# JiaruiFeng/KP-GNN

Measured on AMD Instinct MI355X. Metric: graphs/sec KP-GIN fwd+bwd, ZINC-12k K=8 L=8 h=104, higher is better.
Workload: dtype f32; 1 GPU; ZINC-12k-shaped synthetic molecules, KPGINPlus K=8 L=8 h=104 kernel=spd geometric combine, fwd+bwd+Adam, L1 loss; global_batch=2048, nodes_per_batch=47450, khop_edges_per_batch=1018372, active_pairs_per_batch=1018372, parallelism=dp1, launch=hipGraph replay of fwd+bwd, batches=4 pre-staged batches cycled

## Files before the change

### include/kpgnn.h

```cpp
#ifndef KPGNN_H_
#define KPGNN_H_

#include <stddef.h>
#include <stdint.h>

#ifdef __cplusplus
extern "C" {
#endif

#define KPGNN_ABI_VERSION 1

#define KPGNN_OK 0
#define KPGNN_EINVAL (-1)
#define KPGNN_EHIP (-2)
#define KPGNN_ELIMIT (-3)

typedef void* kpgnn_stream_t;

int kpgnn_abi_version(void);
const char* kpgnn_last_error(void);

int kpgnn_device_info(int* cu_count, int* lds_bytes_per_block, int* wavefront, char* arch, int arch_len);


// ... 124 lines not shown
} kpgnn_agg_fwd_desc;

int kpgnn_aggregate_fwd(const kpgnn_agg_fwd_desc* d, kpgnn_stream_t stream);

typedef struct kpgnn_pull_gather_desc {
    int32_t N, K, D;
    int32_t K_csr;
    const int32_t* n_dyn;
    const int32_t* rowptr;
    const int32_t* col;
    const float* slab[16];
    int64_t slab_sn;
    const float* hinit;
    const float* hinit2;
    float* hout;
} kpgnn_pull_gather_desc;

int kpgnn_khop_pull_gather(const kpgnn_pull_gather_desc* d, kpgnn_stream_t stream);

int64_t kpgnn_agg_lds_launch_count(void);

typedef struct kpgnn_agg_bwd_desc {
    int32_t N, K, D, K_csr, mode, n_code0, n_codek, use_tables;
    const int32_t* rowptr_src;
    const int32_t* col_src;
    const uint16_t* code_src;
    const float* dis;
    const float* g;
    int64_t g_sn, g_sk;
    const float* eps;
// ... 460 lines not shown
```

### kp_gnn_amd/_lib.py

```python
import ctypes
import os

import torch

_PKG = os.path.dirname(os.path.abspath(__file__))
HIP_LIB_PATH = os.path.join(_PKG, "libkpgnn_hip.so")

MODE_GIN, MODE_GINPLUS, MODE_GCN, MODE_SUM = 0, 1, 2, 3

c_i32, c_i64, c_f32p, c_vp = ctypes.c_int32, ctypes.c_int64, ctypes.c_void_p, ctypes.c_void_p


MATH_AUTO, MATH_F32 = 0, 1
ELIMIT = -3
DENSE_MATH = MATH_AUTO


class KpgnnError(RuntimeError):
    pass


class AggFwdDesc(ctypes.Structure):
    _fields_ = [
        ("N", c_i32), ("K", c_i32), ("D", c_i32), ("K_csr", c_i32), ("mode", c_i32),
# ... 6 lines not shown
        ("out", c_vp), ("o_sn", c_i64), ("o_sk", c_i64),
        ("pre", c_vp), ("theta", c_vp), ("hout", c_vp), ("xbias", c_vp),
        ("ptab", c_vp), ("uid", c_vp), ("uid_stride", c_i64),
        ("x_slot", c_vp * 16), ("n_dict", c_i32), ("alphas", c_vp), ("storage", c_i32),
        ("n_dyn", c_vp),
        ("graph_ptr", c_vp), ("num_graphs", c_i32), ("max_graph_nodes", c_i32), ("hinit", c_vp), ("hinit2", c_vp),
    ]


class PullGatherDesc(ctypes.Structure):
    _fields_ = [
        ("N", c_i32), ("K", c_i32), ("D", c_i32), ("K_csr", c_i32),
        ("n_dyn", c_vp), ("rowptr", c_vp), ("col", c_vp),
        ("slab", c_vp * 16), ("slab_sn", c_i64),
        ("hinit", c_vp), ("hinit2", c_vp), ("hout", c_vp),
    ]


class AggBwdDesc(ctypes.Structure):
    _fields_ = [
        ("N", c_i32), ("K", c_i32), ("D", c_i32), ("K_csr", c_i32), ("mode", c_i32),
        ("n_code0", c_i32), ("n_codek", c_i32), ("use_tables", c_i32),
        ("rowptr_src", c_vp), ("col_src", c_vp), ("code_src", c_vp), ("dis", c_vp),
        ("g", c_vp), ("g_sn", c_i64), ("g_sk", c_i64),
        ("eps", c_vp),
        ("gx", c_vp), ("gx_sn", c_i64), ("gx_sk", c_i64),
        ("gtable0", c_vp), ("gtablek", c_vp),
        ("gx_slot", c_vp * 16), ("accumulate_mask", ctypes.c_uint32), ("storage", c_i32),
        ("n_dyn", c_vp),
    ]
# ... 451 lines not shown
```

### kp_gnn_amd/csrc/aggregate.hip

```cpp
#include <initializer_list>

#include "kpgnn_common.h"

namespace kpgnn {
namespace {

constexpr int kBlock = 256;
constexpr int kMaxLdsTableBytes = 96 * 1024;

template <int VEC> struct V {
    float v[VEC];
    __device__ __forceinline__ static V zero() { V r; for (int i = 0; i < VEC; ++i) r.v[i] = 0.f; return r; }
    __device__ __forceinline__ static V load(const float* p) { V r; ldv<VEC>(p, r.v); return r; }
    __device__ __forceinline__ void store(float* p) const { stv<VEC>(p, v); }
    __device__ __forceinline__ void store_stream(float* p) const {
        for (int i = 0; i < VEC; ++i) __builtin_nontemporal_store(v[i], p + i);
    }
    template <bool BF> __device__ __forceinline__ static V load_row(const char* p) {
        if (BF) { V r; ld_bf16<VEC>(p, r.v); return r; }
        return load(reinterpret_cast<const float*>(p));
    }
    __device__ __forceinline__ void add(const V& o) { for (int i = 0; i < VEC; ++i) v[i] += o.v[i]; }
    __device__ __forceinline__ void fma(float s, const V& o) { for (int i = 0; i < VEC; ++i) v[i] = fmaf(s, o.v[i], v[i]); }
};
// ... 16 lines not shown
    const float* periph; int64_t p_sn, p_sk;
    const float* eps;
    float* out; int64_t o_sn, o_sk;
    float* pre;
    const float* theta;
    const float* alphas;
    float* theta_out;
    float* hout;
    const float* hinit;
    const float* hinit2;
    const float* xbias;
    const float* ptab; const int32_t* uid; int64_t uid_stride;
    const float* xs[16];
    int lds_theta, lds_ptab;
};

#ifndef KPGNN_PULL_WAVES
#define KPGNN_PULL_WAVES 7
#endif
#ifndef KPGNN_PULL_PF
#define KPGNN_PULL_PF 4
#endif
template <int VEC, int G, bool GCN, int TAB, bool FAST = false, bool BF = false, bool PULL = false>
__global__ void __launch_bounds__(kBlock, PULL ? KPGNN_PULL_WAVES : FAST ? 5 : 4)
agg_fwd_kernel(const FwdParams p) {
    static_assert(!PULL || (!GCN && TAB == 0 && !FAST && !BF), "the pull form gathers fp32 slabs without tables");
    const int N_live = live_rows(p.N, p.n_dyn);
    const int MODE = PULL ? (int)KPGNN_MODE_SUM : FAST ? (int)KPGNN_MODE_GINPLUS : p.mode;
    const bool COMBINE = (FAST || PULL) ? true : p.combine != 0;
    extern __shared__ __attribute__((aligned(16))) float lds_tab[];
    const int D = p.D;
    const float* thp = p.theta;
    const float* ptp = p.ptab;
    if (TAB == 1) {
        const int n0 = p.n_code0 * D, nk = p.n_codek * D;
        for (int t = threadIdx.x; t < n0; t += kBlock) lds_tab[t] = p.table0[t];
        for (int t = threadIdx.x; t < nk; t += kBlock) lds_tab[n0 + t] = p.tablek[t];
        float* th_l = lds_tab + ((n0 + nk + 3) & ~3);
        float* pt_l = th_l + ((p.lds_theta + 3) & ~3);
        if (p.alphas) {
            for (int d = threadIdx.x; d < D; d += kBlock) {
// ... 11 lines not shown
                    th_l[k * D + d] = th;
                    if (blockIdx.x == 0) p.theta_out[(int64_t)k * D + d] = th;
                    pw *= q;
                }
            }
        } else
        for (int t = threadIdx.x; t < p.lds_theta; t += kBlock) th_l[t] = p.theta[t];
        for (int t = threadIdx.x; t < p.lds_ptab; t += kBlock) pt_l[t] = p.ptab[t];
        if (p.lds_theta) thp = th_l;
        if (p.lds_ptab) ptp = pt_l;
        __syncthreads();
    }
    const float* tab0 = TAB == 1 ? lds_tab : p.table0;
    const float* tabk = TAB == 1 ? lds_tab + p.n_code0 * D : p.tablek;

    constexpr int NODES = kBlock / G;
    const int sg = threadIdx.x / G;
    const int sl = threadIdx.x % G;
    const int lane = threadIdx.x & (kWave - 1);
    const int sg_lane0 = lane - sl;
    const int c0 = sl * VEC;
    const bool col_ok = c0 < D;
    const float eps1 = 1.0f + (!PULL && p.eps ? p.eps[0] : 0.0f);
    const int64_t num_tiles = ((int64_t)N_live + NODES - 1) / NODES;
    constexpr uint32_t XB = BF ? 2u : 4u;
    const uint32_t xrow_b = (uint32_t)p.x_sn * XB, trow_b = (uint32_t)D * 4u;
    const uint32_t lane_b = col_ok ? (uint32_t)c0 * 4u : 0u;
    const uint32_t lane_bx = col_ok ? (uint32_t)c0 * XB : 0u;

    int last_u = -1;
    V<VEC> prow = V<VEC>::zero();
    for (XcdTileWalk w(num_tiles); w.valid(); w.next()) {
        const int64_t i = w.cur * NODES + sg;
        if (i >= N_live) continue;
        const int32_t* rp = p.rowptr + i * p.K_csr;
        V<VEC> hsum = V<VEC>::zero();
        if (!FAST && p.hinit && col_ok) hsum = V<VEC>::load(p.hinit + i * (int64_t)D + c0);
        if (!FAST && p.hinit2 && col_ok) hsum.add(V<VEC>::load(p.hinit2 + i * (int64_t)D + c0));
        const bool lane_meta = PULL ? true : G > p.K;
        int myrp = 0, myuid = 0;
        if (lane_meta) {
            myrp = rp[sl <= p.K ? sl : p.K];
            if (!PULL && (FAST || (p.uid && !p.periph))) myuid = p.uid[i * p.uid_stride + (sl < p.K ? sl : 0)];
        }
        int beg = lane_meta ? __shfl(myrp, sg_lane0) : rp[0];
        const int end_all = lane_meta ? __shfl(myrp, sg_lane0 + p.K) : rp[p.K];
        int cbase = beg;
        uint32_t coff = 0, ctab = 0;
        if (!GCN) {
            const int idx = cbase + sl;
            if (idx < end_all) {
                coff = (uint32_t)p.col[idx] * xrow_b;
                if (TAB != 0) ctab = (uint32_t)p.code[idx] * trow_b;
// ... 149 lines not shown
                if (FAST) v.add(V<VEC>::load(ptp + (int64_t)u * D + c0));
                else { if (u != last_u) { prow = V<VEC>::load(ptp + (int64_t)u * D + c0); last_u = u; } v.add(prow); }
            }
            if (MODE == KPGNN_MODE_GIN) { V<VEC> xs = V<VEC>::load(xk + i * p.x_sn); xs.add(xb); v.fma(eps1, xs); }
            if (COMBINE) {
                if (!FAST && !thp) hsum.add(v);
                else {
                    const V<VEC> th = V<VEC>::load(thp + k * D + c0);
                    for (int q = 0; q < VEC; ++q) hsum.v[q] = fmaf(th.v[q], v.v[q], hsum.v[q]);
                }
            } else {
                v.store_stream(p.out + i * p.o_sn + (int64_t)k * p.o_sk + c0);
            }
        }
        if (COMBINE && col_ok) hsum.store_stream(p.hout + i * (int64_t)D + c0);
    }
}

struct BwdParams {
    const int32_t* n_dyn;
    int N, K, D, K_csr, n_code0, n_codek, mode, bf;
    const int32_t* rowptr;
    const int32_t* col;
    const uint16_t* code;
    const float* dis;
    const float* g; int64_t g_sn, g_sk;
    const float* eps;
    float* gx; int64_t gx_sn, gx_sk;
    float* gtable0;
    float* gtablek;
// ... 183 lines not shown
    }
    if (TAB == 1) {
        __syncthreads();
        for (int t = threadIdx.x; t < n0; t += kBlock) { const float v = lds_gt[t]; if (v != 0.f) atomicAdd(p.gtable0 + t, v); }
        for (int t = threadIdx.x; t < nk; t += kBlock) { const float v = lds_gt[n0 + t]; if (v != 0.f) atomicAdd(p.gtablek + t, v); }
    }
}

unsigned pick_grid(int64_t num_tiles, int blocks_per_cu) {
    const int64_t cap = (int64_t)device_facts().cu_count * blocks_per_cu;
    int64_t g = num_tiles < cap ? num_tiles : cap;
    if (g >= kNumXcd) g = g / kNumXcd * kNumXcd;
    return (unsigned)(g > 0 ? g : 1);
}

template <int VEC, int G, bool GCN, int TAB, bool FAST = false, bool BF = false, bool PULL = false>
int launch_fwd(const FwdParams& p, size_t lds, hipStream_t s) {
    const int64_t tiles = ((int64_t)p.N + (kBlock / G) - 1) / (kBlock / G);
    if (lds > 64 * 1024)
        KPGNN_HIP_TRY(ensure_dynamic_lds((const void*)agg_fwd_kernel<VEC, G, GCN, TAB, FAST, BF, PULL>, lds));
    int nb = resident_blocks(agg_fwd_kernel<VEC, G, GCN, TAB, FAST, BF, PULL>, kBlock, lds);
    if (PULL && nb > KPGNN_PULL_WAVES) nb = KPGNN_PULL_WAVES;
    const unsigned grid = pick_grid(tiles, nb > 0 ? nb : 4);
    hipLaunchKernelGGL((agg_fwd_kernel<VEC, G, GCN, TAB, FAST, BF, PULL>), dim3(grid), dim3(kBlock), lds, s, p);
    KPGNN_LAUNCH_CHECK("agg_fwd_kernel");
    return KPGNN_OK;
}

template <int VEC, int G>
int launch_fwd_mode(const FwdParams& p, int tab, size_t lds, hipStream_t s) {
    const bool gcn = p.mode == KPGNN_MODE_GCN;
    const bool fast = tab == 1 && p.mode == KPGNN_MODE_GINPLUS && p.combine && !p.periph && p.uid && p.ptab && p.pre;
    if (p.bf) {
        if constexpr (VEC == 4) {
            if (fast && !p.x) return launch_fwd<VEC, G, false, 1, true, true>(p, lds, s);
        }
        return fail(KPGNN_EINVAL, "aggregate_fwd: bf16 storage needs the fused KP-GIN+ epilogue (GELU, theta, dictionary P, "
                    "code tables in LDS, S saved), per-hop inputs and D %% 4 == 0");
    }
// ... 132 lines not shown
    return dispatch_row_shape<64>(vec, row_lanes(d->D, vec), "aggregate_fwd",
                                  [&](auto VV, auto G) { return launch_fwd_mode<VV.value, G.value>(p, tab, lds, s); });
}

extern "C" int kpgnn_khop_pull_gather(const kpgnn_pull_gather_desc* d, kpgnn_stream_t stream) {
    KPGNN_REQUIRE(d != nullptr, "khop_pull_gather: NULL descriptor");
    KPGNN_REQUIRE(d->N >= 0 && d->K >= 1 && d->K <= 16 && d->D >= 1 && d->K_csr >= d->K, "khop_pull_gather: bad N=%d K=%d D=%d K_csr=%d",
                  d->N, d->K, d->D, d->K_csr);
    if ((int64_t)d->N * d->K_csr >= ((int64_t)1 << 31)) return fail(KPGNN_ELIMIT, "khop_pull_gather: N*K exceeds int32");
    if (d->N == 0) return KPGNN_OK;
    KPGNN_REQUIRE(d->rowptr != nullptr, "khop_pull_gather: NULL rowptr");
    KPGNN_REQUIRE(d->hout != nullptr, "khop_pull_gather: NULL output");
    for (int k = 0; k < d->K; ++k) KPGNN_REQUIRE(d->slab[k] != nullptr, "khop_pull_gather: NULL slab[%d]", k);
    if ((uint64_t)d->N * (uint64_t)d->slab_sn * 4u >= (1ull << 32))
        return fail(KPGNN_ELIMIT, "khop_pull_gather: N * slab row stride = %lld floats exceeds the 32-bit byte offsets of the gather", (long long)d->N * d->slab_sn);
    FwdParams p = {};
    p.N = d->N; p.n_dyn = d->n_dyn; p.K = d->K; p.D = d->D; p.K_csr = d->K_csr;
    p.mode = KPGNN_MODE_SUM; p.combine = 1;
    p.rowptr = d->rowptr; p.col = d->col;
    p.x_sn = d->slab_sn;
    p.hout = d->hout; p.hinit = d->hinit; p.hinit2 = d->hinit2;
    uintptr_t slot_bits = 0;
    for (int k = 0; k < d->K; ++k) {
        p.xs[k] = d->slab[k];
        slot_bits |= (uintptr_t)p.xs[k] & 15;
    }
    const void* slot_align = (const void*)(slot_bits | 16);
    const int vec = row_vec(d->D, {slot_align, d->hout, d->hinit, d->hinit2}, {d->slab_sn});
    const int lanes = (d->D + vec - 1) / vec;
    if (lanes > 64) return fail(KPGNN_ELIMIT, "khop_pull_gather: D=%d with %d-wide access needs %d lanes > 64", d->D, vec, lanes);
    hipStream_t s = (hipStream_t)stream;
    return dispatch_row_shape<64>(vec, row_lanes(d->D, vec), "khop_pull_gather", [&](auto VV, auto G) {
        if constexpr (VV.value == 4 && G.value >= 16) {
            if (G.value > d->K) return launch_fwd<4, G.value, false, 0, false, false, true>(p, 0, s);
        }
        return launch_fwd<VV.value, G.value, false, 0>(p, 0, s);
    });
}

extern "C" int kpgnn_aggregate_bwd(const kpgnn_agg_bwd_desc* d, kpgnn_stream_t stream) {
    KPGNN_REQUIRE(d != nullptr, "aggregate_bwd: NULL descriptor");
    KPGNN_REQUIRE(d->N >= 0 && d->K >= 1 && d->D >= 1 && d->K_csr >= d->K, "aggregate_bwd: bad N=%d K=%d D=%d K_csr=%d",
                  d->N, d->K, d->D, d->K_csr);
    if ((int64_t)d->N * d->K_csr >= ((int64_t)1 << 31)) return fail(KPGNN_ELIMIT, "aggregate_bwd: N*K exceeds int32");
    if (d->N == 0) return KPGNN_OK;
    KPGNN_REQUIRE(d->rowptr_src && d->g, "aggregate_bwd: NULL rowptr/g");
    if (!d->gx) {
// ... 51 lines not shown
```

### kp_gnn_amd/ops.py

```python
import ctypes

import torch

from . import _lib
from ._lib import MODE_GCN, MODE_GIN, MODE_GINPLUS, MODE_SUM, LaunchTimer, set_launch_timer

_SQRT1_2 = 0.7071067811865476
_INV_SQRT_2PI = 0.3989422804014327


def algorithmic_bytes(csr, k_act, D, n_tensors, n_rows_tables, extra_nd=0, s=4):
    A = csr.active_pairs(k_act)
    return int(s * csr.N * k_act * D * n_tensors) + A * 6 + 4 * (csr.N * csr.K + 1) + 4 * D * n_rows_tables \
        + 4 * csr.N * D * extra_nd


_STORAGE = torch.float32


def set_storage_dtype(dtype):
    global _STORAGE
    prev = _STORAGE
    dtype = {"fp32": torch.float32, "f32": torch.float32, "bf16": torch.bfloat16}.get(dtype, dtype)
    if dtype not in (torch.float32, torch.bfloat16):
# ... 195 lines not shown
        n_t = 1 + (periph is not None) + (pre is not None) + (theta is None)
        extra = 4 * N * K if uid is not None else 0
        return extra + algorithmic_bytes(csr, K, D, n_t, d.n_code0 + d.n_codek, extra_nd=1 if theta is not None else 0,
                                         s=2 if bf16 else 4)
    _lib.launch("kpgnn_aggregate_fwd", dev, ctypes.byref(d), timed=("agg_fwd", nbytes))
    return out, pre


PULL_GATHER = True


def pull_applies(N, D, dtype=torch.float32):
    return PULL_GATHER and dtype == torch.float32 and N >= 4096 and D % 4 == 0


def khop_pull_gather(csr, slabs, hinit, hinit2=None):
    K = len(slabs)
    N, D = slabs[0].shape
    dev = slabs[0].device
    out = hinit if hinit is not None else torch.empty((N, D), dtype=torch.float32, device=dev)
    d = _lib.PullGatherDesc()
    d.N, d.K, d.D, d.K_csr = N, K, D, csr.K
    d.n_dyn = dyn_ptr(N)
    d.rowptr, d.col = csr.rowptr_src.data_ptr(), csr.col_src.data_ptr()
    d.slab_sn = D
    for k, t in enumerate(slabs):
        assert t.shape == (N, D) and t.is_contiguous() and t.dtype == torch.float32
        d.slab[k] = t.data_ptr()
    d.hout, d.hinit, d.hinit2 = out.data_ptr(), _ptr(hinit), _ptr(hinit2)
    _lib.launch("kpgnn_khop_pull_gather", dev, ctypes.byref(d), timed=("agg_bwd", lambda: algorithmic_bytes(
        csr, K, D, 1, 0, extra_nd=1 + (hinit is not None) + (hinit2 is not None))))
    return out


def aggregate_bwd_raw(csr, k_act, mode, g, eps, n_code0, n_codek, want_tables, slots=False, slot_bufs=None, gx_accum=None):
    N, K, D = g.shape
    dev = g.device
    bf16 = g.dtype == torch.bfloat16
    d = _lib.AggBwdDesc()
    d.N, d.K, d.D, d.K_csr, d.mode = N, K, D, csr.K, mode
    d.n_dyn = dyn_ptr(N)
    d.storage = 1 if bf16 else 0
    d.use_tables = 1 if want_tables else 0
    d.n_code0, d.n_codek = n_code0, n_codek
    d.rowptr_src, d.col_src, d.code_src = csr.rowptr_src.data_ptr(), csr.col_src.data_ptr(), csr.code_src.data_ptr()
    d.dis = csr.gcn_dis().data_ptr() if mode == MODE_GCN else None
# ... 503 lines not shown
            top = max(pend) if pend else 0
            zeros = None
            slabs = [g[:, 0]]
            for h in range(1, top + 1):
                t = pend.get(h)
                if t is None:
                    zeros = torch.zeros_like(slabs[0]) if zeros is None else zeros
                    t = zeros
                slabs.append(t)
            hb = c0.buf
            shape = tuple(slabs[0].shape)
            ok = lambda t: t is not None and t.is_contiguous() and t.dtype == torch.float32 and tuple(t.shape) == shape
            hinit = hb if ok(hb) else None
            ext = c0.take_addend()
            hinit2 = ext if ok(ext) else None
            total = khop_pull_gather(csr, slabs[:16], hinit, hinit2)
            if hb is not None and hinit is None:
                total = total + hb.view_as(total)
            if ext is not None and hinit2 is None:
                total = total + ext.view_as(total)
            c0.buf = None
            return (None, gt0, gtk, gperiph, None, _finish_gtheta(ctx, gtheta, theta, galphas_done, k_act), None, gdict, None, None, None,
                    None, None, total, *([None] * (k_act - 1)))
        gx, a0, ak = aggregate_bwd_raw(csr, k_act, mode, g, eps, ctx.n_code0, ctx.n_codek, tables_in_gather,
                                       slots=ctx.n_slots > 0, slot_bufs=_slot_bufs(ctx), gx_accum=xbuf)
        if ctx.n_slots > 0 and ctx.cells is not None:
            ext = ctx.cells[0].take_addend()
            if ext is not None:
                gx = list(gx)
                gx[0] = gx[0] + ext.view_as(gx[0])
            pend = ctx.cells[0].take_slabs()
# ... 28 lines not shown
        galpha = torch.empty_like(ctx.alphas)
        _lib.launch("kpgnn_geo_theta_bwd", galpha.device,
                    ctx.alphas.data_ptr(), theta.data_ptr(), gtheta.data_ptr(), k_act, ctx.alphas.numel(), galpha.data_ptr())
        return galpha
    return gtheta


def _backward_pass_id():
    try:
        return torch._C._current_graph_task_id()
    except AttributeError:
        return -1


class _SlotGradCell:
    __slots__ = ("_buf", "_task", "_pend", "_ptask", "_add", "_atask", "pull_reader", "_dg", "_dgtask")

    def __init__(self):
        self._buf, self._task = None, -1
        self._pend, self._ptask = None, -1
        self._add, self._atask = None, -1
        self.pull_reader = False
        self._dg, self._dgtask = None, -1

    def park_dict(self, uid, theta, gh):
        if self._dg is None or self._dgtask != _backward_pass_id():
            self._dg, self._dgtask = [], _backward_pass_id()
        self._dg.append((uid, theta, gh))

    def take_dicts(self):
        t = self._dg if self._dgtask == _backward_pass_id() else None
        self._dg, self._dgtask = None, -1
        return t or []
# ... 56 lines not shown

def khop_aggregate(x, csr, k_act, mode, table0=None, tablek=None, periph=None, eps=None, theta=None, xbias=None,
                   share_slot_grads=False, x_state=None):
    ptab = uid = None
    if isinstance(periph, DictPeripheral):
        ptab, uid, periph = periph.table, periph.uid, None
    if isinstance(x, (list, tuple)):
        cells = None
        if share_slot_grads and torch.is_grad_enabled():
            cells = []
            for t in x:
                c = getattr(t, "_kp_slot_cell", None)
                if c is None:
                    c = t._kp_slot_cell = _SlotGradCell()
                cells.append(c)
        return KHopAggregate.apply(None, table0, tablek, periph, eps, theta, xbias, ptab, csr, k_act, mode, uid, cells, *x)
    cell = None
    if x_state is not None and torch.is_grad_enabled() and x_state.requires_grad and x_state.is_cuda:
        cell = state_cell(x_state)
    return KHopAggregate.apply(x, table0, tablek, periph, eps, theta, xbias, ptab, csr, k_act, mode, uid, cell)


class DictRows(torch.autograd.Function):

    @staticmethod
    def forward(ctx, table, uid):
        ctx.save_for_backward(uid)
        ctx.n = table.shape[0]
        return table.index_select(0, uid.reshape(-1).long()).view(uid.shape[0], uid.shape[1], table.shape[1])

# ... 390 lines not shown
```

### kp_gnn_amd/ops_dense.py

```python
import ctypes

import torch
import torch.nn.functional as F

from . import _lib
from .ops import _ptr, dyn_ptr, refuse_dynamic_rows


STAT_REPLICAS = 8
_EAGER_DOUBLES = 1 << 20
_GRAPH_DOUBLES = 1 << 18


class _Arena:
    __slots__ = ("buf", "off")

    def __init__(self, n, dev):
        self.buf = torch.zeros(n, dtype=torch.float64, device=dev)
        self.off = 0


_arenas = {}


def take_stat_slot(C, dev):
    lib = _lib.load()
    idx = dev.index if dev.index is not None else torch.cuda.current_device()
    st = _arenas.get(idx)
    if st is None:
        st = _arenas[idx] = {"eager": None, "cap_id": 0, "cap": None}
    cid = ctypes.c_uint64(0)
    _lib.check(lib.kpgnn_stream_capture_id(torch.cuda.current_stream(dev).cuda_stream, ctypes.byref(cid)), "kpgnn_stream_capture_id")
    if cid.value == 0:
        if st["eager"] is None:
            st["eager"] = _Arena(_EAGER_DOUBLES, dev)
        a = st["eager"]
    else:
        if st["cap_id"] != cid.value or st["cap"] is None:
            st["cap"], st["cap_id"] = _Arena(_GRAPH_DOUBLES, dev), cid.value
        a = st["cap"]
    n = (STAT_REPLICAS * 2 * C + 31) // 32 * 32
    if a.off + n > a.buf.numel():
        a.buf.zero_()
        a.off = 0
    v = a.buf[a.off:a.off + n]
    a.off += n
    return v


_COLSTATS = "_kpgnn_colstats"


def attach_column_stats(t, slot):
    try:
        setattr(t, _COLSTATS, (t._version, slot))
    except Exception:
        pass


def _column_stats_of(t):
    rec = getattr(t, _COLSTATS, None)
    if rec is not None and rec[0] == t._version:
# ... 268 lines not shown
    d.n_dyn = dyn_ptr(kw["N"])
    w = kw["w"]
    hit = _split_cache.get((w.data_ptr(), 1 if kw.get("w_transposed", 0) else 0))
    if hit is not None and hit[0] == w._version and hit[1] == kw["O"] and hit[2] == kw["I"]:
        d.workspace, d.workspace_bytes, d.w_split_ready = hit[3].data_ptr(), hit[3].numel(), 1
    else:
        ws = _split_workspace(lib, kw["O"], kw["I"], 1, dev)
        if ws is not None:
            d.workspace, d.workspace_bytes = ws.data_ptr(), ws.numel()
    _lib.launch("kpgnn_linear_bn", dev, ctypes.byref(d))


class FusedMLP(torch.autograd.Function):

    @staticmethod
    def forward(ctx, h, w0, b0, g1, be1, w3, b3, g2, be2, bn1, bn2, out_slot, gO=None, beO=None, residual=None, bnO=None):
        lib = _lib.load()
        dev = h.device
        N, I = h.shape
        O = w0.shape[0]
        h = h.contiguous()
        w0c, w3c = w0.contiguous(), w3.contiguous()
        outer = bnO is not None
        slot1, slot2 = take_stat_slot(O, dev), take_stat_slot(O, dev)
        if outer:
            out_slot = take_stat_slot(O, dev)
        y1 = torch.empty((N, O), dtype=torch.float32, device=dev)
        y2 = torch.empty((N, O), dtype=torch.float32, device=dev)
        st = torch.empty((6, O), dtype=torch.float32, device=dev)
        _lin_bn(lib, dev, N=N, O=O, I=I, x=h, w=w0c, bias=b0, y=y1, pro=0, epi=1, out_slot=slot1)
        track1 = bn1.track_running_stats
        _lin_bn(lib, dev, N=N, O=O, I=O, x=y1, w=w3c, bias=b3, y=y2, pro=1, epi=1, pro_relu=1, in_slot=slot1, in_gamma=g1,
                in_beta=be1, in_eps=float(bn1.eps), momentum=float(bn1.momentum), in_mean=st[0], in_invstd=st[1],
                running_mean=bn1.running_mean if track1 else None, running_var=bn1.running_var if track1 else None,
                num_batches_tracked=bn1.num_batches_tracked if track1 else None, out_slot=slot2)
        d = _lib.BnDesc()
        d.N, d.C, d.relu, d.eps, d.momentum = N, O, 1, float(bn2.eps), float(bn2.momentum)
        d.n_dyn = dyn_ptr(N)
        d.x, d.x_stride, d.gamma, d.beta = y2.data_ptr(), O, g2.data_ptr(), be2.data_ptr()
        if bn2.track_running_stats:
            d.running_mean, d.running_var = bn2.running_mean.data_ptr(), bn2.running_var.data_ptr()
            d.num_batches_tracked = bn2.num_batches_tracked.data_ptr()
        out = torch.empty((N, O), dtype=torch.float32, device=dev)
        d.mean, d.invstd, d.z, d.z_stride = st[2].data_ptr(), st[3].data_ptr(), out.data_ptr(), O
        d.stat_slot, d.stats_ready, d.out_slot = slot2.data_ptr(), 1, _ptr(out_slot)
        ctx.outer, ctx.has_res, ctx.res_cell = outer, False, None
        if outer:
            d.outer_gamma, d.outer_beta = gO.data_ptr(), beO.data_ptr()
            d.outer_eps, d.outer_momentum = float(bnO.eps), float(bnO.momentum)
            if bnO.track_running_stats:
                d.outer_running_mean, d.outer_running_var = bnO.running_mean.data_ptr(), bnO.running_var.data_ptr()
                d.outer_num_batches_tracked = bnO.num_batches_tracked.data_ptr()
            d.outer_mean, d.outer_invstd = st[4].data_ptr(), st[5].data_ptr()
            if residual is not None:
                residual = residual if residual.stride(-1) == 1 else residual.contiguous()
                d.residual, d.r_stride = residual.data_ptr(), residual.stride(0)
                ctx.has_res = True
                ctx.res_cell = getattr(residual, "_kp_slot_cell", None)
        _lib.launch("kpgnn_bn_fwd", dev, ctypes.byref(d))
        if outer:
            ctx.save_for_backward(h, w0c, w3c, g1, be1, g2, be2, y1, y2, st, gO)
# ... 1 lines not shown
            ctx.save_for_backward(h, w0c, w3c, g1, be1, g2, be2, y1, y2, st)
        ctx.has_b0, ctx.has_b3 = b0 is not None, b3 is not None
        return out

    @staticmethod
    def backward(ctx, dz):
        if ctx.outer:
            h, w0, w3, g1, be1, g2, be2, y1, y2, st, gO = ctx.saved_tensors
        else:
            h, w0, w3, g1, be1, g2, be2, y1, y2, st = ctx.saved_tensors
        lib = _lib.load()
        dev = h.device
        N, I = h.shape
        O = w0.shape[0]
        dz = dz.contiguous()
        slot2, slot1 = take_stat_slot(4 * O if ctx.outer else O, dev), take_stat_slot(O, dev)
        dy2 = torch.empty((N, O), dtype=torch.float32, device=dev)
        da1 = torch.empty((N, O), dtype=torch.float32, device=dev)
        dy1 = torch.empty((N, O), dtype=torch.float32, device=dev)
        dh = torch.empty((N, I), dtype=torch.float32, device=dev)
        gb = torch.empty((6, O), dtype=torch.float32, device=dev)
        d = _lib.BnBwdDesc()
        d.N, d.C, d.relu = N, O, 1
        d.n_dyn = dyn_ptr(N)
        d.x, d.x_stride, d.dz, d.dz_stride = y2.data_ptr(), O, dz.data_ptr(), O
        d.gamma, d.beta, d.mean, d.invstd = g2.data_ptr(), be2.data_ptr(), st[2].data_ptr(), st[3].data_ptr()
        d.stat_slot, d.reduce_only = slot2.data_ptr(), 1
        rbuf = None
        handed = False
        if ctx.outer:
            from . import ops
            want_res = ctx.res_cell is not None and ctx.needs_input_grad[14]
            if want_res and ops.pull_applies(N, O) and ctx.res_cell.pull_reader:
                ctx.res_cell.park_addend(dz)
                handed = True
            elif want_res:
                rbuf = ctx.res_cell.buf
            d.outer_mean, d.outer_invstd = st[4].data_ptr(), st[5].data_ptr()
            if rbuf is not None:
                d.residual_grad, d.rg_stride = rbuf.data_ptr(), rbuf.stride(0)
        _lib.launch("kpgnn_bn_bwd", dev, ctypes.byref(d))
        okw = dict(pro=3, o_mean=st[4], o_invstd=st[5], o_gamma=gO, o_dgamma=gb[4], o_dbeta=gb[5]) if ctx.outer else dict(pro=2)
        _lin_bn(lib, dev, N=N, O=O, I=O, x=dz, w=w3, y=da1, w_transposed=1, epi=2, pro_relu=1, in_slot=slot2,
                in_gamma=g2, in_beta=be2, in_mean=st[2], in_invstd=st[3], x2=y2, xt=dy2, dgamma=gb[0], dbeta=gb[1],
                out_slot=slot1, e_x=y1, e_mean=st[0], e_invstd=st[1], e_gamma=g1, e_beta=be1, **okw)
        _lin_bn(lib, dev, N=N, O=I, I=O, x=da1, w=w0, y=dh, w_transposed=1, pro=2, epi=0, pro_relu=0, in_slot=slot1,
                in_gamma=g1, in_beta=be1, in_mean=st[0], in_invstd=st[1], x2=y1, xt=dy1, dgamma=gb[2], dbeta=gb[3])
        dw3 = torch.empty((O, O), dtype=torch.float32, device=dev)
        dw0 = torch.empty((O, I), dtype=torch.float32, device=dev)
        db = torch.empty((2, O), dtype=torch.float32, device=dev)
        a, b = _lib.WgradDesc(), _lib.WgradDesc()
        a.N, a.O, a.I = N, O, O
        a.n_dyn = b.n_dyn = dyn_ptr(N)
        a.dy, a.dy_stride, a.x, a.x_stride = dy2.data_ptr(), O, y1.data_ptr(), O
        a.dw, a.db = dw3.data_ptr(), db[0].data_ptr()
        a.x_mean, a.x_invstd, a.x_gamma, a.x_beta, a.x_relu = st[0].data_ptr(), st[1].data_ptr(), g1.data_ptr(), be1.data_ptr(), 1
# ... 8 lines not shown
            job = ops.defer_reduce_job(w0, w3)
            if job is not None:
                a.defer = ctypes.cast(ctypes.pointer(job), ctypes.c_void_p)
            _lib.launch("kpgnn_linear_wgrad_pair", dev, ctypes.byref(a), ctypes.byref(b))
            if job is not None:
                ops.queue_reduce_job(job, (ws, dw3, dw0, db))
        else:
            for q in (a, b):
                nb = int(lib.kpgnn_wgrad_workspace_bytes(q.O, q.I))
                ws = torch.empty(nb, dtype=torch.uint8, device=dev)
                q.workspace, q.workspace_bytes = ws.data_ptr(), nb
                _lib.launch("kpgnn_linear_wgrad", dev, ctypes.byref(q))
        gres = dz if (ctx.outer and ctx.has_res and rbuf is None and not handed) else None
        return (dh if ctx.needs_input_grad[0] else None, dw0, db[1] if ctx.has_b0 else None, gb[2], gb[3],
                dw3, db[0] if ctx.has_b3 else None, gb[0], gb[1], None, None, None,
                gb[4] if ctx.outer else None, gb[5] if ctx.outer else None, gres, None)


def _fusable_bn(bn):
    return bn.training and bn.affine and bn.momentum is not None


def mlp_linear_bn_relu_x2(mlp, h, emit_out_stats=False, post_norm=None):
    l0, bn1, l3, bn2 = mlp[0], mlp[1], mlp[3], mlp[4]
    O, I = l0.weight.shape
    bnO, res = post_norm if post_norm is not None else (None, None)
    if (not torch.is_grad_enabled() and h.is_cuda and h.dim() == 2 and h.dtype == torch.float32 and h.shape[0] >= 1
            and _eval_bn(bn1) and _eval_bn(bn2) and (bnO is None or _eval_bn(bnO)) and tuple(l3.weight.shape) == (O, O)
            and _eval_residual_ok(res, (h.shape[0], O))):
        z = mlp_eval_raw(mlp, h, post_norm=post_norm)
        if z is not None:
            return z
        z = batch_norm_act(_eval_linear(h, l0), bn1, relu=True)
        z = batch_norm_act(_eval_linear(z, l3), bn2, relu=True)
        return z if bnO is None else batch_norm_act(z, bnO, relu=False, residual=res)
    if (h.is_cuda and h.dim() == 2 and h.dtype == torch.float32 and torch.is_grad_enabled() and _fusable_bn(bn1)
            and _fusable_bn(bn2) and I in _LIN_WIDTHS and O in _LIN_WIDTHS and tuple(l3.weight.shape) == (O, O)
            and h.shape[0] >= 1 and h.data_ptr() % 16 == 0
            and (l0.bias is None or l0.bias.data_ptr() % 16 == 0) and (l3.bias is None or l3.bias.data_ptr() % 16 == 0)):
        if (bnO is not None and _fusable_bn(bnO) and bnO.weight.data_ptr() % 16 == 0 and bnO.bias.data_ptr() % 16 == 0
                and (res is None or (res.is_cuda and res.dtype == torch.float32 and tuple(res.shape) == (h.shape[0], O)
                                     and res.stride(0) % 4 == 0 and res.data_ptr() % 16 == 0))):
            return FusedMLP.apply(h, l0.weight, l0.bias, bn1.weight, bn1.bias, l3.weight, l3.bias, bn2.weight, bn2.bias,
                                  bn1, bn2, None, bnO.weight, bnO.bias, res, bnO)
        out_slot = take_stat_slot(O, h.device) if (emit_out_stats or bnO is not None) else None
        z = FusedMLP.apply(h, l0.weight, l0.bias, bn1.weight, bn1.bias, l3.weight, l3.bias, bn2.weight, bn2.bias, bn1, bn2,
                           out_slot)
        if out_slot is not None:
            attach_column_stats(z, out_slot)
    else:
        z = batch_norm_act(linear(h, mlp[0]), mlp[1], relu=True)
        z = batch_norm_act(linear(z, mlp[3]), mlp[4], relu=True)
    return z if bnO is None else batch_norm_act(z, bnO, relu=False, residual=res)


def _jk_native_ok(weight, bias, states, forward_only=False):
    S = len(states)
    N, H = states[0].shape
    O = weight.shape[0]
# ... 404 lines not shown
```

Measured before the change: 672,300 graphs/s.

## Fuse BatchNorm backward column reductions into the k-hop pull-gather kernel

Measured after the change: 671,400 graphs/s. Within noise of the previous version (-0.1%).

```diff
diff --git a/include/kpgnn.h b/include/kpgnn.h
--- a/include/kpgnn.h
+++ b/include/kpgnn.h
@@ -162,6 +162,11 @@
     const float* hinit;
     const float* hinit2;
     float* hout;
+    const float* y; int64_t y_stride;
+    const float* mean; const float* invstd; const float* gamma; const float* beta;
+    const float* outer_mean; const float* outer_invstd;
+    int32_t relu;
+    double* stat_slot;
 } kpgnn_pull_gather_desc;
 
 int kpgnn_khop_pull_gather(const kpgnn_pull_gather_desc* d, kpgnn_stream_t stream);
diff --git a/kp_gnn_amd/_lib.py b/kp_gnn_amd/_lib.py
--- a/kp_gnn_amd/_lib.py
+++ b/kp_gnn_amd/_lib.py
@@ -44,6 +44,9 @@
         ("n_dyn", c_vp), ("rowptr", c_vp), ("col", c_vp),
         ("slab", c_vp * 16), ("slab_sn", c_i64),
         ("hinit", c_vp), ("hinit2", c_vp), ("hout", c_vp),
+        ("y", c_vp), ("y_stride", c_i64),
+        ("mean", c_vp), ("invstd", c_vp), ("gamma", c_vp), ("beta", c_vp), ("outer_mean", c_vp), ("outer_invstd", c_vp),
+        ("relu", c_i32), ("stat_slot", c_vp),
     ]
 
 
diff --git a/kp_gnn_amd/csrc/aggregate.hip b/kp_gnn_amd/csrc/aggregate.hip
--- a/kp_gnn_amd/csrc/aggregate.hip
+++ b/kp_gnn_amd/csrc/aggregate.hip
@@ -54,6 +54,19 @@
     const float* xs[16];
     int lds_theta, lds_ptab;
 };
+struct StatsParams : FwdParams {
+    const float* s_y; int64_t s_ys;
+    const float* s_mean; const float* s_invstd; const float* s_gamma; const float* s_beta;
+    const float* s_omean; const float* s_oinvstd;
+    int s_relu;
+    double* s_slot;
+};
+template <bool STATS> using ParamsOf = std::conditional_t<STATS, StatsParams, FwdParams>;
+
+template <typename T, int N> __device__ __forceinline__ T* stats_lds() {
+    __shared__ __attribute__((aligned(16))) T a[N];
+    return a;
+}
 
 #ifndef KPGNN_PULL_WAVES
 #define KPGNN_PULL_WAVES 7
@@ -61,10 +74,19 @@
 #ifndef KPGNN_PULL_PF
 #define KPGNN_PULL_PF 4
 #endif
-template <int VEC, int G, bool GCN, int TAB, bool FAST = false, bool BF = false, bool PULL = false>
-__global__ void __launch_bounds__(kBlock, PULL ? KPGNN_PULL_WAVES : FAST ? 5 : 4)
-agg_fwd_kernel(const FwdParams p) {
+#ifndef KPGNN_PULLSTATS_BLOCK
+#define KPGNN_PULLSTATS_BLOCK 1024
+#endif
+#ifndef KPGNN_PULLSTATS_WAVES
+#define KPGNN_PULLSTATS_WAVES 4
+#endif
+constexpr int kStatsRun = 16;
+template <int VEC, int G, bool GCN, int TAB, bool FAST = false, bool BF = false, bool PULL = false, bool STATS = false>
+__global__ void __launch_bounds__(STATS ? KPGNN_PULLSTATS_BLOCK : kBlock, STATS ? KPGNN_PULLSTATS_WAVES : PULL ? KPGNN_PULL_WAVES : FAST ? 5 : 4)
+agg_fwd_kernel(const ParamsOf<STATS> p) {
     static_assert(!PULL || (!GCN && TAB == 0 && !FAST && !BF), "the pull form gathers fp32 slabs without tables");
+    static_assert(!STATS || PULL, "the BatchNorm sums ride with the pull form only");
+    constexpr int BLK = STATS ? KPGNN_PULLSTATS_BLOCK : kBlock;
     const int N_live = live_rows(p.N, p.n_dyn);
     const int MODE = PULL ? (int)KPGNN_MODE_SUM : FAST ? (int)KPGNN_MODE_GINPLUS : p.mode;
     const bool COMBINE = (FAST || PULL) ? true : p.combine != 0;
@@ -106,7 +128,7 @@
     const float* tab0 = TAB == 1 ? lds_tab : p.table0;
     const float* tabk = TAB == 1 ? lds_tab + p.n_code0 * D : p.tablek;
 
-    constexpr int NODES = kBlock / G;
+    constexpr int NODES = BLK / G;
     const int sg = threadIdx.x / G;
     const int sl = threadIdx.x % G;
     const int lane = threadIdx.x & (kWave - 1);
@@ -114,6 +136,35 @@
     const int c0 = sl * VEC;
     const bool col_ok = c0 < D;
     const float eps1 = 1.0f + (!PULL && p.eps ? p.eps[0] : 0.0f);
+    constexpr int GV = G * VEC;
+    double* sacc = nullptr;
+    const float* scst = nullptr;
+    float ta[STATS ? 8 : 1][VEC];
+    int nacc = 0;
+    if constexpr (STATS) {
+        sacc = stats_lds<double, 8 * GV>();
+        float* c = stats_lds<float, 6 * GV>();
+        for (int t = threadIdx.x; t < 8 * GV; t += BLK) sacc[t] = 0.0;
+        for (int t = threadIdx.x; t < GV; t += BLK) {
+            const bool ok = t < D;
+            c[0 * GV + t] = ok ? p.s_mean[t] : 0.f;  c[1 * GV + t] = ok ? p.s_invstd[t] : 0.f;
+            c[2 * GV + t] = ok ? p.s_gamma[t] : 0.f; c[3 * GV + t] = ok ? p.s_beta[t] : 0.f;
+            c[4 * GV + t] = ok ? p.s_omean[t] : 0.f; c[5 * GV + t] = ok ? p.s_oinvstd[t] : 0.f;
+        }
+        for (int n = 0; n < 8; ++n) for (int q = 0; q < VEC; ++q) ta[n][q] = 0.f;
+        __syncthreads();
+        scst = c;
+    }
+    auto stats_flush = [&]() {
+        if constexpr (STATS) {
+            if (col_ok) {
+#pragma unroll
+                for (int n = 0; n < 8; ++n)
+                    for (int q = 0; q < VEC; ++q) { atomicAdd(sacc + n * GV + c0 + q, (double)ta[n][q]); ta[n][q] = 0.f; }
+            }
+            nacc = 0;
+        }
+    };
     const int64_t num_tiles = ((int64_t)N_live + NODES - 1) / NODES;
     constexpr uint32_t XB = BF ? 2u : 4u;
     const uint32_t xrow_b = (uint32_t)p.x_sn * XB, trow_b = (uint32_t)D * 4u;
@@ -129,6 +180,8 @@
         V<VEC> hsum = V<VEC>::zero();
         if (!FAST && p.hinit && col_ok) hsum = V<VEC>::load(p.hinit + i * (int64_t)D + c0);
         if (!FAST && p.hinit2 && col_ok) hsum.add(V<VEC>::load(p.hinit2 + i * (int64_t)D + c0));
+        V<VEC> yrow = V<VEC>::zero();
+        if constexpr (STATS) { if (col_ok) yrow = V<VEC>::load(p.s_y + i * p.s_ys + c0); }
         const bool lane_meta = PULL ? true : G > p.K;
         int myrp = 0, myuid = 0;
         if (lane_meta) {
@@ -308,6 +361,44 @@
             }
         }
         if (COMBINE && col_ok) hsum.store_stream(p.hout + i * (int64_t)D + c0);
+        if constexpr (STATS) {
+            if (col_ok) {
+                const V<VEC> mean = V<VEC>::load(scst + 0 * GV + c0), istd = V<VEC>::load(scst + 1 * GV + c0);
+                const V<VEC> gm = V<VEC>::load(scst + 2 * GV + c0), bt = V<VEC>::load(scst + 3 * GV + c0);
+                const V<VEC> om = V<VEC>::load(scst + 4 * GV + c0), oi = V<VEC>::load(scst + 5 * GV + c0);
+                for (int q = 0; q < VEC; ++q) {
+                    const float xi = (yrow.v[q] - mean.v[q]) * istd.v[q];
+                    const float pre = fmaf(xi, gm.v[q], bt.v[q]);
+                    const bool m = !p.s_relu || pre > 0.f;
+                    const float z = (p.s_relu && pre <= 0.f) ? 0.f : pre;
+                    const float xo = (z - om.v[q]) * oi.v[q];
+                    const float d = hsum.v[q];
+                    ta[0][q] += d;
+                    ta[1][q] = fmaf(d, xo, ta[1][q]);
+                    if (m) {
+                        ta[2][q] += d;
+                        ta[3][q] += 1.0f;
+                        ta[4][q] += xo;
+                        ta[5][q] = fmaf(d, xi, ta[5][q]);
+                        ta[6][q] += xi;
+                        ta[7][q] = fmaf(xo, xi, ta[7][q]);
+                    }
+                }
+            }
+            if (++nacc == kStatsRun) stats_flush();
+        }
+    }
+    if constexpr (STATS) {
+        if (nacc) stats_flush();
+        __syncthreads();
+        double* slot = p.s_slot + (int64_t)(blockIdx.x % KPGNN_STAT_REPLICAS) * 8 * D;
+        for (int t = threadIdx.x; t < 8 * GV; t += BLK) {
+            const int n = t / GV, col = t - n * GV;
+            if (col < D) {
+                const double v = sacc[t];
+                if (v != 0.0) atomicAdd(slot + (int64_t)n * D + col, v);
+            }
+        }
     }
 }
 
@@ -521,15 +612,19 @@
     return (unsigned)(g > 0 ? g : 1);
 }
 
-template <int VEC, int G, bool GCN, int TAB, bool FAST = false, bool BF = false, bool PULL = false>
-int launch_fwd(const FwdParams& p, size_t lds, hipStream_t s) {
-    const int64_t tiles = ((int64_t)p.N + (kBlock / G) - 1) / (kBlock / G);
+template <int VEC, int G, bool GCN, int TAB, bool FAST = false, bool BF = false, bool PULL = false, bool STATS = false>
+int launch_fwd(const ParamsOf<STATS>& p, size_t lds, hipStream_t s) {
+    constexpr int BLK = STATS ? KPGNN_PULLSTATS_BLOCK : kBlock;
+    const int64_t tiles = ((int64_t)p.N + (BLK / G) - 1) / (BLK / G);
     if (lds > 64 * 1024)
-        KPGNN_HIP_TRY(ensure_dynamic_lds((const void*)agg_fwd_kernel<VEC, G, GCN, TAB, FAST, BF, PULL>, lds));
-    int nb = resident_blocks(agg_fwd_kernel<VEC, G, GCN, TAB, FAST, BF, PULL>, kBlock, lds);
-    if (PULL && nb > KPGNN_PULL_WAVES) nb = KPGNN_PULL_WAVES;
+        KPGNN_HIP_TRY(ensure_dynamic_lds((const void*)agg_fwd_kernel<VEC, G, GCN, TAB, FAST, BF, PULL, STATS>, lds));
+    int nb = resident_blocks(agg_fwd_kernel<VEC, G, GCN, TAB, FAST, BF, PULL, STATS>, BLK, lds);
+    if (PULL && !STATS && nb > KPGNN_PULL_WAVES) nb = KPGNN_PULL_WAVES;
+    constexpr int kStatsBlocks = KPGNN_PULLSTATS_WAVES * 256 / KPGNN_PULLSTATS_BLOCK;
+    static_assert(kStatsBlocks >= 1, "KPGNN_PULLSTATS_WAVES holds less than one block per CU");
+    if (STATS && (nb <= 0 || nb > kStatsBlocks)) nb = kStatsBlocks;
     const unsigned grid = pick_grid(tiles, nb > 0 ? nb : 4);
-    hipLaunchKernelGGL((agg_fwd_kernel<VEC, G, GCN, TAB, FAST, BF, PULL>), dim3(grid), dim3(kBlock), lds, s, p);
+    hipLaunchKernelGGL((agg_fwd_kernel<VEC, G, GCN, TAB, FAST, BF, PULL, STATS>), dim3(grid), dim3(BLK), lds, s, p);
     KPGNN_LAUNCH_CHECK("agg_fwd_kernel");
     return KPGNN_OK;
 }
@@ -692,7 +787,7 @@
     for (int k = 0; k < d->K; ++k) KPGNN_REQUIRE(d->slab[k] != nullptr, "khop_pull_gather: NULL slab[%d]", k);
     if ((uint64_t)d->N * (uint64_t)d->slab_sn * 4u >= (1ull << 32))
         return fail(KPGNN_ELIMIT, "khop_pull_gather: N * slab row stride = %lld floats exceeds the 32-bit byte offsets of the gather", (long long)d->N * d->slab_sn);
-    FwdParams p = {};
+    StatsParams p = {};
     p.N = d->N; p.n_dyn = d->n_dyn; p.K = d->K; p.D = d->D; p.K_csr = d->K_csr;
     p.mode = KPGNN_MODE_SUM; p.combine = 1;
     p.rowptr = d->rowptr; p.col = d->col;
@@ -704,11 +799,30 @@
         slot_bits |= (uintptr_t)p.xs[k] & 15;
     }
     const void* slot_align = (const void*)(slot_bits | 16);
+    const bool stats = d->y || d->stat_slot || d->mean || d->invstd || d->gamma || d->beta || d->outer_mean || d->outer_invstd;
+    if (stats) {
+        KPGNN_REQUIRE(d->y && d->stat_slot && d->mean && d->invstd && d->gamma && d->beta && d->outer_mean && d->outer_invstd,
+                      "khop_pull_gather: the stats block needs y, mean, invstd, gamma, beta, outer_mean, outer_invstd and stat_slot");
+        KPGNN_REQUIRE(d->y_stride >= d->D, "khop_pull_gather: y_stride=%lld < D=%d", (long long)d->y_stride, d->D);
+        KPGNN_REQUIRE(((uintptr_t)d->stat_slot & 7) == 0, "khop_pull_gather: stat_slot is not 8-byte aligned");
+        for (const void* q : {(const void*)d->y, (const void*)d->mean, (const void*)d->invstd, (const void*)d->gamma, (const void*)d->beta,
+                              (const void*)d->outer_mean, (const void*)d->outer_invstd})
+            KPGNN_REQUIRE(((uintptr_t)q & 15) == 0, "khop_pull_gather: the stats block's rows must be 16-byte aligned");
+        KPGNN_REQUIRE(d->y_stride % 4 == 0, "khop_pull_gather: y_stride=%lld is not a multiple of 4", (long long)d->y_stride);
+        p.s_y = d->y; p.s_ys = d->y_stride; p.s_mean = d->mean; p.s_invstd = d->invstd; p.s_gamma = d->gamma; p.s_beta = d->beta;
+        p.s_omean = d->outer_mean; p.s_oinvstd = d->outer_invstd; p.s_relu = d->relu ? 1 : 0; p.s_slot = d->stat_slot;
+    }
     const int vec = row_vec(d->D, {slot_align, d->hout, d->hinit, d->hinit2}, {d->slab_sn});
     const int lanes = (d->D + vec - 1) / vec;
     if (lanes > 64) return fail(KPGNN_ELIMIT, "khop_pull_gather: D=%d with %d-wide access needs %d lanes > 64", d->D, vec, lanes);
     hipStream_t s = (hipStream_t)stream;
     return dispatch_row_shape<64>(vec, row_lanes(d->D, vec), "khop_pull_gather", [&](auto VV, auto G) {
+        if constexpr (VV.value == 4 && G.value == 32) {
+            if (stats && G.value > d->K) return launch_fwd<4, G.value, false, 0, false, false, true, true>(p, 0, s);
+        }
+        if (stats)
+            return fail(KPGNN_ELIMIT, "khop_pull_gather: the stats block needs D %% 4 == 0, 68 <= D <= 128, 16-byte aligned operands and "
+                        "K < 32 (D=%d, %d-wide access, K=%d): run kpgnn_bn_bwd's stacked reduce instead", d->D, VV.value * 4, d->K);
         if constexpr (VV.value == 4 && G.value >= 16) {
             if (G.value > d->K) return launch_fwd<4, G.value, false, 0, false, false, true>(p, 0, s);
         }
diff --git a/kp_gnn_amd/ops.py b/kp_gnn_amd/ops.py
--- a/kp_gnn_amd/ops.py
+++ b/kp_gnn_amd/ops.py
@@ -233,7 +233,35 @@
     return PULL_GATHER and dtype == torch.float32 and N >= 4096 and D % 4 == 0
 
 
-def khop_pull_gather(csr, slabs, hinit, hinit2=None):
+PULL_STATS = True
+
+
+class PullStats:
+    __slots__ = ("y", "st", "gamma", "beta", "relu", "slot", "dh", "task", "epoch")
+
+    def __init__(self, relu=True):
+        self.y = self.st = self.gamma = self.beta = None
+        self.relu = relu
+        self.slot = self.dh = self.epoch = None
+        self.task = -1
+
+    def ready(self, shape):
+        y = self.y
+        return (y is not None and tuple(y.shape) == tuple(shape) and y.is_contiguous() and y.dtype == torch.float32
+                and 68 <= shape[1] <= 128 and shape[1] % 4 == 0 and y.data_ptr() % 16 == 0 and self.st.data_ptr() % 16 == 0
+                and self.gamma.data_ptr() % 16 == 0 and self.beta.data_ptr() % 16 == 0)
+
+    def take(self, dz):
+        slot, dh, task, epoch = self.slot, self.dh, self.task, self.epoch
+        self.slot = self.dh = self.epoch = None
+        self.task = -1
+        if (slot is None or dh is None or task != _backward_pass_id() or dz.data_ptr() != dh.data_ptr()
+                or tuple(dz.shape) != tuple(dh.shape) or not dz.is_contiguous()):
+            return None, None
+        return slot, epoch
+
+
+def khop_pull_gather(csr, slabs, hinit, hinit2=None, stats=None, stat_slot=None):
     K = len(slabs)
     N, D = slabs[0].shape
     dev = slabs[0].device
@@ -247,8 +275,14 @@
         assert t.shape == (N, D) and t.is_contiguous() and t.dtype == torch.float32
         d.slab[k] = t.data_ptr()
     d.hout, d.hinit, d.hinit2 = out.data_ptr(), _ptr(hinit), _ptr(hinit2)
+    if stats is not None:
+        st = stats.st
+        d.y, d.y_stride = stats.y.data_ptr(), stats.y.stride(0)
+        d.mean, d.invstd, d.outer_mean, d.outer_invstd = st[2].data_ptr(), st[3].data_ptr(), st[4].data_ptr(), st[5].data_ptr()
+        d.gamma, d.beta, d.relu = stats.gamma.data_ptr(), stats.beta.data_ptr(), 1 if stats.relu else 0
+        d.stat_slot = stat_slot.data_ptr()
     _lib.launch("kpgnn_khop_pull_gather", dev, ctypes.byref(d), timed=("agg_bwd", lambda: algorithmic_bytes(
-        csr, K, D, 1, 0, extra_nd=1 + (hinit is not None) + (hinit2 is not None))))
+        csr, K, D, 1, 0, extra_nd=1 + (hinit is not None) + (hinit2 is not None) + (stats is not None))))
     return out
 
 
@@ -782,7 +816,17 @@
             hinit = hb if ok(hb) else None
             ext = c0.take_addend()
             hinit2 = ext if ok(ext) else None
-            total = khop_pull_gather(csr, slabs[:16], hinit, hinit2)
+            req = c0.stats_src if PULL_STATS else None
+            slot = None
+            if (req is not None and req.ready(shape) and (hb is None or hinit is not None) and (ext is None or hinit2 is not None)
+                    and all(t.data_ptr() % 16 == 0 for t in slabs[:16]) and (hinit is None or hinit.data_ptr() % 16 == 0)
+                    and (hinit2 is None or hinit2.data_ptr() % 16 == 0)):
+                from .ops_dense import stat_slot_epoch, take_stat_slot
+                slot = take_stat_slot(4 * shape[1], slabs[0].device)
+                epoch = stat_slot_epoch(slabs[0].device)
+            total = khop_pull_gather(csr, slabs[:16], hinit, hinit2, stats=req if slot is not None else None, stat_slot=slot)
+            if slot is not None:
+                req.slot, req.dh, req.task, req.epoch = slot, total, _backward_pass_id(), epoch
             if hb is not None and hinit is None:
                 total = total + hb.view_as(total)
             if ext is not None and hinit2 is None:
@@ -841,9 +885,10 @@
 
 
 class _SlotGradCell:
-    __slots__ = ("_buf", "_task", "_pend", "_ptask", "_add", "_atask", "pull_reader", "_dg", "_dgtask")
+    __slots__ = ("_buf", "_task", "_pend", "_ptask", "_add", "_atask", "pull_reader", "_dg", "_dgtask", "stats_src")
 
     def __init__(self):
+        self.stats_src = None
         self._buf, self._task = None, -1
         self._pend, self._ptask = None, -1
         self._add, self._atask = None, -1
@@ -930,6 +975,8 @@
                 if c is None:
                     c = t._kp_slot_cell = _SlotGradCell()
                 cells.append(c)
+            if cells:
+                cells[0].stats_src = getattr(x[0], "_kp_pull_stats", None)
         return KHopAggregate.apply(None, table0, tablek, periph, eps, theta, xbias, ptab, csr, k_act, mode, uid, cells, *x)
     cell = None
     if x_state is not None and torch.is_grad_enabled() and x_state.requires_grad and x_state.is_cuda:
diff --git a/kp_gnn_amd/ops_dense.py b/kp_gnn_amd/ops_dense.py
--- a/kp_gnn_amd/ops_dense.py
+++ b/kp_gnn_amd/ops_dense.py
@@ -13,17 +13,30 @@
 
 
 class _Arena:
-    __slots__ = ("buf", "off")
+    __slots__ = ("buf", "off", "gen")
 
     def __init__(self, n, dev):
         self.buf = torch.zeros(n, dtype=torch.float64, device=dev)
         self.off = 0
+        self.gen = 0
 
 
 _arenas = {}
 
 
 def take_stat_slot(C, dev):
+    a = _arena_of(dev)
+    n = (STAT_REPLICAS * 2 * C + 31) // 32 * 32
+    if a.off + n > a.buf.numel():
+        a.buf.zero_()
+        a.off = 0
+        a.gen += 1
+    v = a.buf[a.off:a.off + n]
+    a.off += n
+    return v
+
+
+def _arena_of(dev):
     lib = _lib.load()
     idx = dev.index if dev.index is not None else torch.cuda.current_device()
     st = _arenas.get(idx)
@@ -34,18 +47,15 @@
     if cid.value == 0:
         if st["eager"] is None:
             st["eager"] = _Arena(_EAGER_DOUBLES, dev)
-        a = st["eager"]
-    else:
-        if st["cap_id"] != cid.value or st["cap"] is None:
-            st["cap"], st["cap_id"] = _Arena(_GRAPH_DOUBLES, dev), cid.value
-        a = st["cap"]
-    n = (STAT_REPLICAS * 2 * C + 31) // 32 * 32
-    if a.off + n > a.buf.numel():
-        a.buf.zero_()
-        a.off = 0
-    v = a.buf[a.off:a.off + n]
-    a.off += n
-    return v
+        return st["eager"]
+    if st["cap_id"] != cid.value or st["cap"] is None:
+        st["cap"], st["cap_id"] = _Arena(_GRAPH_DOUBLES, dev), cid.value
+    return st["cap"]
+
+
+def stat_slot_epoch(dev):
+    a = _arena_of(dev)
+    return (a, a.gen)
 
 
 _COLSTATS = "_kpgnn_colstats"
@@ -344,7 +354,8 @@
 class FusedMLP(torch.autograd.Function):
 
     @staticmethod
-    def forward(ctx, h, w0, b0, g1, be1, w3, b3, g2, be2, bn1, bn2, out_slot, gO=None, beO=None, residual=None, bnO=None):
+    def forward(ctx, h, w0, b0, g1, be1, w3, b3, g2, be2, bn1, bn2, out_slot, gO=None, beO=None, residual=None, bnO=None,
+                stats_req=None):
         lib = _lib.load()
         dev = h.device
         N, I = h.shape
@@ -375,6 +386,9 @@
         d.mean, d.invstd, d.z, d.z_stride = st[2].data_ptr(), st[3].data_ptr(), out.data_ptr(), O
         d.stat_slot, d.stats_ready, d.out_slot = slot2.data_ptr(), 1, _ptr(out_slot)
         ctx.outer, ctx.has_res, ctx.res_cell = outer, False, None
+        ctx.stats_req = stats_req if outer else None
+        if ctx.stats_req is not None:
+            stats_req.y, stats_req.st, stats_req.gamma, stats_req.beta, stats_req.relu = y2, st, g2, be2, True
         if outer:
             d.outer_gamma, d.outer_beta = gO.data_ptr(), beO.data_ptr()
             d.outer_eps, d.outer_momentum = float(bnO.eps), float(bnO.momentum)
@@ -406,7 +420,6 @@
         N, I = h.shape
         O = w0.shape[0]
         dz = dz.contiguous()
-        slot2, slot1 = take_stat_slot(4 * O if ctx.outer else O, dev), take_stat_slot(O, dev)
         dy2 = torch.empty((N, O), dtype=torch.float32, device=dev)
         da1 = torch.empty((N, O), dtype=torch.float32, device=dev)
         dy1 = torch.empty((N, O), dtype=torch.float32, device=dev)
@@ -417,7 +430,7 @@
         d.n_dyn = dyn_ptr(N)
         d.x, d.x_stride, d.dz, d.dz_stride = y2.data_ptr(), O, dz.data_ptr(), O
         d.gamma, d.beta, d.mean, d.invstd = g2.data_ptr(), be2.data_ptr(), st[2].data_ptr(), st[3].data_ptr()
-        d.stat_slot, d.reduce_only = slot2.data_ptr(), 1
+        d.reduce_only = 1
         rbuf = None
         handed = False
         if ctx.outer:
@@ -431,7 +444,19 @@
             d.outer_mean, d.outer_invstd = st[4].data_ptr(), st[5].data_ptr()
             if rbuf is not None:
                 d.residual_grad, d.rg_stride = rbuf.data_ptr(), rbuf.stride(0)
-        _lib.launch("kpgnn_bn_bwd", dev, ctypes.byref(d))
+        slot2 = slot1 = None
+        if ctx.stats_req is not None:
+            ready, epoch = ctx.stats_req.take(dz)
+            if ready is not None and rbuf is None:
+                slot1 = take_stat_slot(O, dev)
+                a, gen = stat_slot_epoch(dev)
+                if a is epoch[0] and gen == epoch[1]:
+                    slot2 = ready
+        if slot2 is None:
+            slot2 = take_stat_slot(4 * O if ctx.outer else O, dev)
+            slot1 = take_stat_slot(O, dev) if slot1 is None else slot1
+            d.stat_slot = slot2.data_ptr()
+            _lib.launch("kpgnn_bn_bwd", dev, ctypes.byref(d))
         okw = dict(pro=3, o_mean=st[4], o_invstd=st[5], o_gamma=gO, o_dgamma=gb[4], o_dbeta=gb[5]) if ctx.outer else dict(pro=2)
         _lin_bn(lib, dev, N=N, O=O, I=O, x=dz, w=w3, y=da1, w_transposed=1, epi=2, pro_relu=1, in_slot=slot2,
                 in_gamma=g2, in_beta=be2, in_mean=st[2], in_invstd=st[3], x2=y2, xt=dy2, dgamma=gb[0], dbeta=gb[1],
@@ -470,7 +495,7 @@
         gres = dz if (ctx.outer and ctx.has_res and rbuf is None and not handed) else None
         return (dh if ctx.needs_input_grad[0] else None, dw0, db[1] if ctx.has_b0 else None, gb[2], gb[3],
                 dw3, db[0] if ctx.has_b3 else None, gb[0], gb[1], None, None, None,
-                gb[4] if ctx.outer else None, gb[5] if ctx.outer else None, gres, None)
+                gb[4] if ctx.outer else None, gb[5] if ctx.outer else None, gres, None, None)
 
 
 def _fusable_bn(bn):
@@ -497,8 +522,13 @@
         if (bnO is not None and _fusable_bn(bnO) and bnO.weight.data_ptr() % 16 == 0 and bnO.bias.data_ptr() % 16 == 0
                 and (res is None or (res.is_cuda and res.dtype == torch.float32 and tuple(res.shape) == (h.shape[0], O)
                                      and res.stride(0) % 4 == 0 and res.data_ptr() % 16 == 0))):
-            return FusedMLP.apply(h, l0.weight, l0.bias, bn1.weight, bn1.bias, l3.weight, l3.bias, bn2.weight, bn2.bias,
-                                  bn1, bn2, None, bnO.weight, bnO.bias, res, bnO)
+            from . import ops
+            req = ops.PullStats() if (ops.PULL_STATS and ops.pull_applies(h.shape[0], O) and 68 <= O <= 128) else None
+            z = FusedMLP.apply(h, l0.weight, l0.bias, bn1.weight, bn1.bias, l3.weight, l3.bias, bn2.weight, bn2.bias,
+                               bn1, bn2, None, bnO.weight, bnO.bias, res, bnO, req)
+            if req is not None:
+                z._kp_pull_stats = req
+            return z
         out_slot = take_stat_slot(O, h.device) if (emit_out_stats or bnO is not None) else None
         z = FusedMLP.apply(h, l0.weight, l0.bias, bn1.weight, bn1.bias, l3.weight, l3.bias, bn2.weight, bn2.bias, bn1, bn2,
                            out_slot)
```
